# YichengDWu/tinyedm

Measured on AMD Instinct MI355X. Metric: train imgs/sec CIFAR-10 32x32 bf16, higher is better.
Workload: dtype bf16; 1 GPU; CIFAR-10 32x32 unconditional EDM2 U-Net (conf/cifar10.yaml, 35.6M params) full training step: diffuse+embed+denoiser fwd/bwd+loss+grad all-reduce+Adam+EMA; per_gpu_batch=128, global_batch=128, parallelism=dp1, conditional=False, step_launch=hipGraph replay, collective=none

## Files before the change

### tinyedm_amd/csrc/conv_wgrad3.hip

```cpp
#include "common.h"
#include <stdlib.h>

namespace {

typedef const __attribute__((address_space(1))) void* gptr_t;
typedef __attribute__((address_space(3))) void* lptr_t;
typedef __attribute__((address_space(3))) char lds_char;
typedef __attribute__((ext_vector_type(2))) unsigned u32x2_t;

constexpr int KP = 64;
constexpr int SUBB = KP * 64;
constexpr int TCO = 128, TCI = 64;
constexpr int TILE_FLOATS = 9 * TCO * TCI;
constexpr int MAXL = 48;
constexpr int DYRING = 3;

template <int LEADS>
struct Ring {
  static constexpr int XR = LEADS == 1 ? 4 : 8;
  static constexpr int MIRR = LEADS == 1 ? 2 : 4;
  static constexpr int XSLOTS = XR + MIRR;
  static constexpr size_t LDS = (size_t)DYRING * 4 * SUBB + (size_t)2 * XSLOTS * SUBB;
};

// ... 228 lines not shown
            kp = kpp; sw = wp; sh = hp; sn = np_;
            pix = pixel(valid);
            kq = kp;
            kp = kpn; sw = wn; sh = hn; sn = nn;
          }
          valid = valid && kq < ks1;
#pragma unroll
          for (int sub = 0; sub < 4; ++sub)
            if (valid && co0 + sub * 32 < Cout) dsrc[sub] = dY + pix * Cout + co0 + sub * 32 + dp * 8;
        }
      }
      char* const xdst = Xb + xslot * SUBB + wave * 1024;
      char* const ddst = dYb + ((t + 2) % DYRING) * (4 * SUBB) + wave * 1024;
      if constexpr (MF16) {
        const int slot = (t + LEADS) & (XR - 1);
        const int base_row = (slot < LEADS ? slot + XR : slot) * KP;
        const unsigned a_u = (unsigned)(uintptr_t)(lds_char*)dYb + (t % DYRING) * (4 * SUBB) + (cb * 2) * SUBB + krow16 * 64 + chan16;
        const unsigned b_u = (unsigned)(uintptr_t)(lds_char*)Xb + ib * (XSLOTS * SUBB) + (base_row + krow16) * 64 + chan16;
        unsigned tb[9];
#pragma unroll
        for (int tp = 0; tp < 9; ++tp) tb[tp] = b_u + ((tp / 3 - 1) * PW + (tp % 3 - 1)) * 64;
        u32x2_t A[2][4][2], Bf[6][2];
#define A_RD(set, c, ks2_)                                                                    \
  TR_RD(A[set][c][0], a_u, ((c) >> 1) * SUBB + ((c) & 1) * 32 + (ks2_) * 2048);               \
  TR_RD(A[set][c][1], a_u, ((c) >> 1) * SUBB + ((c) & 1) * 32 + (ks2_) * 2048 + 256);
        A_RD(0, 0, 0) A_RD(0, 1, 0) A_RD(0, 2, 0) A_RD(0, 3, 0)
        TR_RD(Bf[0][0], tb[0], 0); TR_RD(Bf[0][1], tb[0], 256);
        TR_RD(Bf[1][0], tb[0], 32); TR_RD(Bf[1][1], tb[0], 32 + 256);
        TR_RD(Bf[2][0], tb[1], 0); TR_RD(Bf[2][1], tb[1], 256);
        static_for<0, 36>([&](auto nc) {
          constexpr int n = decltype(nc)::value;
          constexpr int ks2 = n / 18, f = n % 18, tp = f / 2, b = f % 2;
          const unsigned au_ = a_u;
          constexpr int na = ((n - 3 <= 8 && 8 <= n - 1) ? 1 : 0) + ((n - 3 <= 10 && 10 <= n - 1) ? 1 : 0) +
                             ((n - 3 <= 12 && 12 <= n - 1) ? 1 : 0) + ((n - 3 <= 14 && 14 <= n - 1) ? 1 : 0);
          constexpr int cnt = n >= 33 ? (35 - n) * 2 : 4 + 2 * na;
          asm volatile("s_waitcnt lgkmcnt(%0)" ::"n"(cnt) : "memory");
          __builtin_amdgcn_sched_barrier(0);
          if constexpr (n == 1) { if (do_x) { dma16(xsrc0, xdst); if (xslot < MIRR) dma16(xsrc0, xdst + XR * SUBB); } __builtin_amdgcn_sched_barrier(0); }
          if constexpr (n == 5) { if (do_x) { dma16(xsrc1, xdst + XSLOTS * SUBB); if (xslot < MIRR) dma16(xsrc1, xdst + (XSLOTS + XR) * SUBB); } __builtin_amdgcn_sched_barrier(0); }
          if constexpr (n == 10) { if (do_dy) dma16(dsrc[0], ddst); __builtin_amdgcn_sched_barrier(0); }
          if constexpr (n == 14) { if (do_dy) dma16(dsrc[1], ddst + SUBB); __builtin_amdgcn_sched_barrier(0); }
          if constexpr (n == 19) { if (do_dy) dma16(dsrc[2], ddst + 2 * SUBB); __builtin_amdgcn_sched_barrier(0); }
          if constexpr (n == 23) { if (do_dy) dma16(dsrc[3], ddst + 3 * SUBB); __builtin_amdgcn_sched_barrier(0); }
          const bf16x8 bfr = frag_of(Bf[n % 6][0], Bf[n % 6][1]);
#pragma unroll
          for (int c = 0; c < 4; ++c) {
            const bf16x8 afr = frag_of(A[ks2 & 1][c][0], A[ks2 & 1][c][1]);
            if constexpr (tp < 8) asm volatile("v_mfma_f32_16x16x32_bf16 %0, %1, %2, %0" : "+a"(acc16[c][b][tp < 8 ? tp : 0]) : "v"(afr), "v"(bfr));
            else asm volatile("v_mfma_f32_16x16x32_bf16 %0, %1, %2, %0" : "+v"(accv16[c][b]) : "v"(afr), "v"(bfr));
            if constexpr (n + 3 < 36) {
              constexpr int m = n + 3, ksm = m / 18, fm = m % 18;
              if (c < 2) TR_RD(Bf[m % 6][c < 2 ? c : 0], tb[fm / 2], ksm * 2048 + (fm % 2) * 32 + (c < 2 ? c : 0) * 256);
            }
          }
          if constexpr (ks2 == 0 && b == 0 && tp >= 4 && tp <= 7) {
            constexpr int ca = tp - 4;
            TR_RD(A[1][ca][0], au_, (ca >> 1) * SUBB + (ca & 1) * 32 + 2048);
            TR_RD(A[1][ca][1], au_, (ca >> 1) * SUBB + (ca & 1) * 32 + 2048 + 256);
          }
        });
#undef A_RD
      } else if constexpr (!(ABL & 8)) {
        const int slot = (t + LEADS) & (XR - 1);
        const int base_row = (slot < LEADS ? slot + XR : slot) * KP;
        unsigned a_u = (unsigned)(uintptr_t)(lds_char*)dYb + (t % DYRING) * (4 * SUBB) + (cb * 2) * SUBB + krow_l * 64 + chan_b;
        const unsigned b_u = (unsigned)(uintptr_t)(lds_char*)Xb + ib * (XSLOTS * SUBB) + (base_row + krow_l) * 64 + chan_b;
        unsigned tb[9];
#pragma unroll
        for (int tp = 0; tp < 9; ++tp) tb[tp] = b_u + ((tp / 3 - 1) * PW + (tp % 3 - 1)) * 64;
        u32x2_t A[2][2][2], Bf[6][2];
        TR_RD(A[0][0][0], a_u, 0); TR_RD(A[0][0][1], a_u, 256);
        TR_RD(A[0][1][0], a_u, SUBB); TR_RD(A[0][1][1], a_u, SUBB + 256);
        TR_RD(Bf[0][0], tb[0], 0); TR_RD(Bf[0][1], tb[0], 256);
        TR_RD(Bf[1][0], tb[1], 0); TR_RD(Bf[1][1], tb[1], 256);
        TR_RD(Bf[2][0], tb[2], 0); TR_RD(Bf[2][1], tb[2], 256);
        static_for<0, 36>([&](auto nc) {
          constexpr int n = decltype(nc)::value;
          constexpr int ks = n / 9, p = n % 9;
          const unsigned au_ = a_u;
          constexpr int cnt = ks < 3 ? (p == 5 || p == 8 ? 6 : (p == 6 || p == 7 ? 8 : 4))
                                     : (p <= 6 ? 4 : (p == 7 ? 2 : 0));
          if constexpr (!(ABL & 32)) asm volatile("s_waitcnt lgkmcnt(%0)" ::"n"(cnt) : "memory");
          __builtin_amdgcn_sched_barrier(0);
          if constexpr (n == 1) { if (do_x) { dma16(xsrc0, xdst); if (xslot < MIRR) dma16(xsrc0, xdst + XR * SUBB); } __builtin_amdgcn_sched_barrier(0); }
          if constexpr (n == 5) { if (do_x) { dma16(xsrc1, xdst + XSLOTS * SUBB); if (xslot < MIRR) dma16(xsrc1, xdst + (XSLOTS + XR) * SUBB); } __builtin_amdgcn_sched_barrier(0); }
          if constexpr (n == 10) { if (do_dy) dma16(dsrc[0], ddst); __builtin_amdgcn_sched_barrier(0); }
          if constexpr (n == 14) { if (do_dy) dma16(dsrc[1], ddst + SUBB); __builtin_amdgcn_sched_barrier(0); }
          if constexpr (n == 19) { if (do_dy) dma16(dsrc[2], ddst + 2 * SUBB); __builtin_amdgcn_sched_barrier(0); }
          if constexpr (n == 23) { if (do_dy) dma16(dsrc[3], ddst + 3 * SUBB); __builtin_amdgcn_sched_barrier(0); }
          const bf16x8 bfr = frag_of(Bf[n % 6][0], Bf[n % 6][1]);
#pragma unroll
          for (int i = 0; i < 2; ++i) {
            const bf16x8 afr = frag_of(A[ks & 1][i][0], A[ks & 1][i][1]);
            if constexpr (!(ABL & 1)) {
              if constexpr (p < 8) asm volatile("v_mfma_f32_32x32x16_bf16 %0, %1, %2, %0" : "+a"(acc[i][p < 8 ? p : 0]) : "v"(afr), "v"(bfr));
              else asm volatile("v_mfma_f32_32x32x16_bf16 %0, %1, %2, %0" : "+v"(accv[i]) : "v"(afr), "v"(bfr));
            }
            if constexpr (n + 3 < 36) {
              constexpr int m = n + 3;
              TR_RD(Bf[m % 6][i], tb[m % 9], (m / 9) * 1024 + i * 256);
            }
          }
          if constexpr (ks < 3 && (p == 4 || p == 5)) {
            constexpr int ia = p - 4;
            TR_RD(A[(ks + 1) & 1][ia][0], au_, ia * SUBB + (ks + 1) * 1024);
            TR_RD(A[(ks + 1) & 1][ia][1], au_, ia * SUBB + (ks + 1) * 1024 + 256);
          }
        });
      } else {
        if (do_x) { dma16(xsrc0, xdst); if (xslot < MIRR) dma16(xsrc0, xdst + XR * SUBB); dma16(xsrc1, xdst + XSLOTS * SUBB); if (xslot < MIRR) dma16(xsrc1, xdst + (XSLOTS + XR) * SUBB); }
        if (do_dy) { dma16(dsrc[0], ddst); dma16(dsrc[1], ddst + SUBB); dma16(dsrc[2], ddst + 2 * SUBB); dma16(dsrc[3], ddst + 3 * SUBB); }
      }
    }
    asm volatile("s_nop 15\n\ts_nop 15" ::: "memory");
    if constexpr (MF16) {
#pragma unroll
      for (int c = 0; c < 4; ++c)
#pragma unroll
        for (int b = 0; b < 2; ++b)
#pragma unroll
          for (int tp = 0; tp < 9; ++tp) {
            float* base = out + ((long)tp * TCO + cb * 64 + c * 16 + 4 * lq) * TCI + ib * 32 + b * 16 + l15;
#pragma unroll
            for (int r = 0; r < 4; ++r) base[r * TCI] = (tp < 8) ? acc16[c][b][tp < 8 ? tp : 0][r] : accv16[c][b][r];
          }
    } else {
#pragma unroll
    for (int i = 0; i < 2; ++i)
#pragma unroll
      for (int tp = 0; tp < 9; ++tp) {
        float* base = out + ((long)tp * TCO + cb * 64 + i * 32) * TCI + ib * 32 + l31;
#pragma unroll
        for (int r = 0; r < 16; ++r)
          base[((r & 3) + 8 * (r >> 2) + 4 * lhi) * TCI] = (tp < 8) ? acc[i][tp < 8 ? tp : 0][r] : accv[i][r];
      }
    }
    pos += nst;
    if (pos >= g.L[li].stage0 + (long)g.L[li].ngroups * g.L[li].nst) ++li;
    __builtin_amdgcn_s_barrier();
  }
}

struct F3Layer {
  const float* w;
  float* grad;
  const int* perm;
  int O, I, Cin, tiles_ci, nst, row0;
  int gci, gco, nblk_ci, group0;
  int ksplit, tiles_co;
  float scale;
  int accumulate;
  long stage0;
};
struct F3Group {
  F3Layer L[MAXL];
  int nlayers, slots_per_member;
  long q;
  const float* work;
};

__device__ __forceinline__ float block_sum_f(float v, float* red) {
  v = wave_sum(v);
  const int lane = threadIdx.x & 63, wave = threadIdx.x >> 6;
  __syncthreads();
  if (lane == 0) red[wave] = v;
  __syncthreads();
  float s = 0.f;
  for (int i = 0; i < (int)(blockDim.x >> 6); ++i) s += red[i];
  return s;
}

__global__ __launch_bounds__(256) void k_wgrad3_finish(const F3Group* __restrict__ gp) {
  const F3Group& g = *gp;
  extern __shared__ __attribute__((aligned(16))) float gsm[];
  __shared__ float red[8];
  int li = 0;
  {
    int hi = g.nlayers - 1;
    while (li < hi) {
      const int mid = (li + hi + 1) >> 1;
      if ((int)blockIdx.x >= g.L[mid].row0) li = mid;
      else hi = mid - 1;
    }
  }
  const int r = blockIdx.x - g.L[li].row0;
  const int I = g.L[li].I, tiles_ci = g.L[li].tiles_ci, nst = g.L[li].nst;
  const int n = I * 9;
  const int mo = g.L[li].perm ? g.L[li].perm[r] : r;
  const float* __restrict__ row = g.L[li].w + (long)mo * n;
  const int tco = r / TCO, rl = r - tco * TCO;
  const float scale = g.L[li].scale;
  constexpr int WPF = 28;
  const bool pf = n <= WPF * 256;
  float wpre[WPF];
  if (pf) {
#pragma unroll
    for (int k = 0; k < WPF; ++k) {
      const int e = threadIdx.x + k * 256;
      wpre[k] = e < n ? row[e] : 0.f;
    }
  }
  const int items = tiles_ci * 9 * 16;
  for (int idx = threadIdx.x; idx < items; idx += blockDim.x) {
    const int c4 = idx & 15, tt = idx >> 4;
    const int tp = tt % 9, tci = tt / 9;
    const int gco = g.L[li].gco, gci = g.L[li].gci, ksplit = g.L[li].ksplit;
    f32x4 a = {0.f, 0.f, 0.f, 0.f};
    for (int ksh = 0; ksh < ksplit; ++ksh) {
      int grp, member;
      if (ksplit > 1) {
        const int v = ksh * (g.L[li].tiles_co * tiles_ci) + tco * tiles_ci + tci;
        grp = v >> 3;
        member = v & 7;
      } else {
        grp = (tco / gco) * g.L[li].nblk_ci + tci / gci;
        member = (tco % gco) * gci + tci % gci;
      }
      const long s0 = g.L[li].stage0 + (long)grp * nst;
      const int w_lo = (int)(s0 / g.q), w_hi = (int)((s0 + nst - 1) / g.q);
      const float* p = g.work + ((long)member * g.slots_per_member + w_lo + g.L[li].group0 + grp) * TILE_FLOATS +
                       ((long)tp * TCO + rl) * TCI + c4 * 4;
      for (int w = w_lo; w <= w_hi; ++w) {
        a += *reinterpret_cast<const f32x4*>(p);
        p += TILE_FLOATS;
      }
    }
    const int i0 = tci * TCI + c4 * 4;
#pragma unroll
    for (int j = 0; j < 4; ++j)
      if (i0 + j < I) gsm[(i0 + j) * 9 + tp] = a[j] * scale;
  }
  __syncthreads();
  float dot = 0.f, ss = 0.f;
  if (pf) {
#pragma unroll
    for (int k = 0; k < WPF; ++k) {
      const int e = threadIdx.x + k * 256;
      if (e < n) {
        dot += gsm[e] * wpre[k];
        ss += wpre[k] * wpre[k];
      }
    }
  } else {
    for (int e = threadIdx.x; e < n; e += blockDim.x) {
      const float wv = row[e];
      dot += gsm[e] * wv;
      ss += wv * wv;
    }
  }
  dot = block_sum_f(dot, red);
  ss = block_sum_f(ss, red);
  const float rn = sqrtf(ss);
  const float sqn = sqrtf((float)n);
  const float d = NORM_EPS + rn / sqn;
  const float c0 = 1.0f / (d * sqn);
  const float c1 = rn > 0.f ? dot / (d * rn * sqn) : 0.f;
  float* __restrict__ outp = g.L[li].grad + (long)mo * n;
  const int accumulate = g.L[li].accumulate;
  if (pf) {
#pragma unroll
    for (int k = 0; k < WPF; ++k) {
      const int e = threadIdx.x + k * 256;
      if (e < n) {
        const float v = c0 * (gsm[e] - wpre[k] * c1);
        outp[e] = accumulate ? outp[e] + v : v;
      }
    }
  } else {
    for (int e = threadIdx.x; e < n; e += blockDim.x) {
      const float v = c0 * (gsm[e] - row[e] * c1);
      outp[e] = accumulate ? outp[e] + v : v;
    }
  }
}

struct Plan {
  W3Group wg;
  F3Group fg;
  int leads, rows_total, ngroups_total, max_n;
  long work_floats;
};

}

extern "C" {
typedef struct {
  const void* X;
  const void* dY;
  const float* w;
  float* grad;
  const int* perm;
  int B, H, W, Cin, Cout, I;
  float scale;
  int accumulate;
} edm_wgrad3_item;
}


namespace {

int make_plan(const edm_wgrad3_item* it, int n, Plan& P) {
  EDM_REQUIRE(it && n > 0 && n <= MAXL, "wgrad3: need 1..%d layers per group, got %d", MAXL, n);
  P.leads = 0;
  long stage = 0;
  int group = 0, row = 0;
  P.max_n = 0;
  for (int k = 0; k < n; ++k) {
    const edm_wgrad3_item& a = it[k];
    EDM_REQUIRE(a.X && a.dY && a.w && a.grad, "wgrad3: null pointer in layer %d", k);
    EDM_REQUIRE(a.B > 0 && a.H > 0 && a.W > 0 && (long)a.B * (a.H + 1) * (a.W + 1) < (1L << 30), "wgrad3: bad B/H/W");
    EDM_REQUIRE(a.Cin > 0 && a.Cin % 32 == 0 && a.Cout > 0 && a.Cout % 32 == 0 && a.I > 0 && a.I <= a.Cin,
                "wgrad3: Cin=%d Cout=%d must be multiples of 32 (I=%d <= Cin)", a.Cin, a.Cout, a.I);
    EDM_REQUIRE(a.W + 2 <= 2 * KP, "wgrad3: W=%d > %d unsupported", a.W, 2 * KP - 2);
    EDM_REQUIRE((long)a.I * 9 * 4 <= 64 * 1024, "wgrad3: fan_in %d too large for the LDS row buffer", a.I * 9);
    const int leads = (a.W + 2 > KP) ? 2 : 1;
    EDM_REQUIRE(P.leads == 0 || P.leads == leads, "wgrad3: layers of one group must share the halo class (W <= 62 or W > 62)");
    P.leads = leads;
    W3Layer& L = P.wg.L[k];
    L.X = (const bf16*)a.X;
    L.dY = (const bf16*)a.dY;
    L.B = a.B; L.H = a.H; L.W = a.W; L.Cin = a.Cin; L.Cout = a.Cout;
    L.PW = a.W + 1;
    L.PH = a.H + 1;
    L.lead_rows = 2 + (leads * KP + L.PW - 1) / L.PW;
    L.kmult = (L.lead_rows + L.PH - 1) / L.PH;
    L.kbeg0 = (long)(L.lead_rows - 1) * L.PW + 1;
    L.kend = ((long)L.lead_rows + (long)a.B * L.PH) * L.PW;
    L.tiles_ci = (a.Cin + TCI - 1) / TCI;
    L.tiles_co = (a.Cout + TCO - 1) / TCO;
    L.gco = L.tiles_co >= 8 ? 8 : L.tiles_co >= 4 ? 4 : L.tiles_co >= 2 ? 2 : 1;
    {
      auto slots = [&](int gco) {
        const int gci = 8 / gco;
        return ((L.tiles_co + gco - 1) / gco) * ((L.tiles_ci + gci - 1) / gci);
      };
      static const bool search = [] { const char* e = getenv("EDM_W3_TEAMS"); return !(e && e[0] == '0'); }();
      int best = L.gco;
      for (int gco = 1; search && gco <= 8; gco *= 2)
        if (slots(gco) < slots(best)) best = gco;
      L.gco = best;
    }
    L.gci = 8 / L.gco;
    L.nblk_ci = (L.tiles_ci + L.gci - 1) / L.gci;
    L.ngroups = ((L.tiles_co + L.gco - 1) / L.gco) * L.nblk_ci;
    L.group0 = group;
    L.nst = (int)((L.kend - L.kbeg0 + KP - 1) / KP);
    L.ksplit = 1;
    {
      constexpr int W3_FLUSH_STAGES = 16;
      static const int smax = [] { const char* e = getenv("EDM_W3_KSPLIT"); return e ? atoi(e) : 8; }();
      const int T = L.tiles_co * L.tiles_ci;
      long best = (long)L.ngroups * (L.nst + W3_FLUSH_STAGES);
      for (int sp = 2; sp <= smax && sp <= 8; ++sp) {
        const int nst_s = (L.nst + sp - 1) / sp;
        if (nst_s < W3_FLUSH_STAGES) break;
        const long cost = (long)((T * sp + 7) / 8) * (nst_s + W3_FLUSH_STAGES);
        if (cost < best) { best = cost; L.ksplit = sp; }
      }
      if (L.ksplit > 1) {
        L.ngroups = (T * L.ksplit + 7) / 8;
        L.nst = (L.nst + L.ksplit - 1) / L.ksplit;
      }
    }
    L.stage0 = stage;
    F3Layer& F = P.fg.L[k];
    F.w = a.w; F.grad = a.grad; F.perm = a.perm;
    F.O = a.Cout; F.I = a.I; F.Cin = a.Cin; F.tiles_ci = L.tiles_ci; F.nst = L.nst; F.row0 = row;
    F.gci = L.gci; F.gco = L.gco; F.nblk_ci = L.nblk_ci; F.group0 = group;
    F.ksplit = L.ksplit; F.tiles_co = L.tiles_co;
    F.scale = a.scale; F.accumulate = a.accumulate; F.stage0 = stage;
    stage += (long)L.ngroups * L.nst;
    group += L.ngroups;
    row += a.Cout;
    if (a.I * 9 > P.max_n) P.max_n = a.I * 9;
  }
  constexpr int NXCD = 8, TPX_MAX = 4, QMIN = 8;
  int tpx = TPX_MAX;
  while (tpx > 1 && stage < (long)QMIN * NXCD * tpx) --tpx;
  const int teams = NXCD * tpx;
  const long q = (stage + teams - 1) / teams;
  P.wg.nlayers = P.fg.nlayers = n;
  P.wg.nwg = teams * 8;
  P.wg.tpx = tpx;
  P.wg.slots_per_member = P.fg.slots_per_member = teams + group;
  P.wg.total = stage;
  P.wg.q = P.fg.q = q;
  P.rows_total = row;
  P.ngroups_total = group;
  P.work_floats = (long)8 * (teams + group) * TILE_FLOATS;
  return EDM_OK;
}

}

extern "C" long edm_wgrad3_workspace(const edm_wgrad3_item* items, int n) {
  Plan P;
  if (make_plan(items, n, P) != EDM_OK) return -1;
  return P.work_floats * 4;
}

extern "C" int edm_wgrad3_plan_ksplit(const edm_wgrad3_item* items, int n, int* ksplit_out) {
  Plan P;
  const int rc = make_plan(items, n, P);
  if (rc != EDM_OK) return rc;
  EDM_REQUIRE(ksplit_out, "wgrad3_plan_ksplit: null output");
  for (int k = 0; k < n; ++k) ksplit_out[k] = P.wg.L[k].ksplit;
  return EDM_OK;
}

extern "C" long edm_wgrad3_table_bytes(void) { return (long)(sizeof(W3Group) + sizeof(F3Group)); }
extern "C" int edm_wgrad3_max_layers(void) { return MAXL; }

static thread_local hipEvent_t g_probe_start = nullptr, g_probe_end = nullptr;
extern "C" int edm_wgrad3_probe(void* ev_start, void* ev_end) {
  g_probe_start = (hipEvent_t)ev_start;
  g_probe_end = (hipEvent_t)ev_end;
  return EDM_OK;
}

extern "C" int edm_wgrad3_group(const edm_wgrad3_item* items, int n, void* workspace, long workspace_bytes,
                                void* table_host, void* table_dev, int defer_upload, hipStream_t st) {
  Plan P;
  const int rc = make_plan(items, n, P);
  if (rc != EDM_OK) return rc;
  EDM_REQUIRE(workspace && workspace_bytes >= P.work_floats * 4, "wgrad3: workspace too small (%ld < %ld bytes)",
              workspace_bytes, P.work_floats * 4);
  const bf16* zeros = (const bf16*)edm_zero_page();
  EDM_REQUIRE(zeros, "wgrad3: edm_init() has not been called on this device");
  P.wg.work = (float*)workspace;
  P.wg.zeros = zeros;
  P.fg.work = (const float*)workspace;
  static_assert(sizeof(W3Group) % 16 == 0, "F3Group must start aligned behind W3Group");
  {
    char stage[sizeof(W3Group) + sizeof(F3Group)];
    memcpy(stage, &P.wg, sizeof(W3Group));
    memcpy(stage + sizeof(W3Group), &P.fg, sizeof(F3Group));
    EDM_UPLOAD_TABLE(table_dev, table_host, stage, sizeof(stage), st, "wgrad3", defer_upload);
  }
  const W3Group* const wgp = (const W3Group*)table_dev;
  const F3Group* const fgp = (const F3Group*)((const char*)table_dev + sizeof(W3Group));
  static std::atomic<unsigned long long> set1{0}, set2{0};
  static const int abl = [] { const char* e = getenv("EDM_W3_ABLATE"); return e ? atoi(e) : 0; }();
  if (g_probe_start) (void)hipEventRecord(g_probe_start, st);
  if (P.leads == 1 && abl) {
    auto go = [&](auto kern) {
      (void)hipFuncSetAttribute(reinterpret_cast<const void*>(kern), hipFuncAttributeMaxDynamicSharedMemorySize, 160 * 1024);
      hipLaunchKernelGGL(kern, dim3(P.wg.nwg), dim3(256), Ring<1>::LDS, st, wgp);
    };
    switch (abl) {
      case 1: go(k_wgrad3<1, 1>); break;
      case 2: go(k_wgrad3<1, 2>); break;
      case 4: go(k_wgrad3<1, 4>); break;
      case 6: go(k_wgrad3<1, 6>); break;
      case 8: go(k_wgrad3<1, 8>); break;
      case 10: go(k_wgrad3<1, 10>); break;
      case 16: go(k_wgrad3<1, 16>); break;
      case 34: go(k_wgrad3<1, 34>); break;
      case 38: go(k_wgrad3<1, 38>); break;
      case 18: go(k_wgrad3<1, 18>); break;
      case 22: go(k_wgrad3<1, 22>); break;
      default: go(k_wgrad3<1, 14>); break;
    }
  } else {
    static const int mf16 = [] { const char* e = getenv("EDM_W3_MFMA16"); return e ? atoi(e) : 1; }();
    auto go = [&](auto kern, size_t lds, std::atomic<unsigned long long>& once) {
      edm_max_lds_once(reinterpret_cast<const void*>(kern), 160 * 1024, once);
      hipLaunchKernelGGL(kern, dim3(P.wg.nwg), dim3(256), lds, st, wgp);
    };
    static std::atomic<unsigned long long> set1m{0}, set2m{0};
    if (P.leads == 1) { if (mf16) go(k_wgrad3<1, 0, true>, Ring<1>::LDS, set1m); else go(k_wgrad3<1>, Ring<1>::LDS, set1); }
    else { if (mf16) go(k_wgrad3<2, 0, true>, Ring<2>::LDS, set2m); else go(k_wgrad3<2>, Ring<2>::LDS, set2); }
  }
  if (g_probe_end) (void)hipEventRecord(g_probe_end, st);
  g_probe_start = g_probe_end = nullptr;
  EDM_CHECK_LAUNCH("wgrad3");
  EDM_MAX_LDS(k_wgrad3_finish, 64 * 1024);
  hipLaunchKernelGGL(k_wgrad3_finish, dim3(P.rows_total), dim3(256), (size_t)P.max_n * 4, st, fgp);
  EDM_CHECK_LAUNCH("wgrad3_finish");
  return EDM_OK;
}
```

### tinyedm_amd/csrc/weights.hip

```cpp
#include "common.h"

namespace {

__device__ __forceinline__ float block_sum(float v, float* red) {
  v = wave_sum(v);
  const int lane = threadIdx.x & 63, wave = threadIdx.x >> 6;
  __syncthreads();
  if (lane == 0) red[wave] = v;
  __syncthreads();
  float s = 0.f;
  for (int i = 0; i < (int)(blockDim.x >> 6); ++i) s += red[i];
  return s;
}

__device__ __forceinline__ void prep_row(float* __restrict__ w, int O, int I, int taps, int Ipad,
                                         bf16* __restrict__ wp_fwd, bf16* __restrict__ wp_dgrad,
                                         float* __restrict__ w_hat, const int* __restrict__ perm,
                                         int normalize_inplace, int r, float* red) {
  const int mo = perm ? perm[r] : r;
  const int n = I * taps;
  float* row = w + (long)mo * n;
  const float rsn = rsqrtf((float)n);
  float ss = 0.f;
  for (int e = threadIdx.x; e < n; e += blockDim.x) ss += row[e] * row[e];
// ... 211 lines not shown
      const int o0 = r0 + og * 8;
      const int c = o0 >> 5, ks = (o0 >> 4) & 1, g = (o0 >> 3) & 1;
      const bf16* src = tile + (long)(og * 8) * n + (long)i * taps + t;
      bf16x8 v;
#pragma unroll
      for (int e = 0; e < 8; ++e) v[e] = src[(long)e * n];
      bf16* dst = d.dgrad + ((((long)((taps - 1 - t) * NC + c) * NCB + (i >> 5)) * 2 + ks) * 64 + g * 32 + (i & 31)) * 8;
      *reinterpret_cast<bf16x8*>(dst) = v;
    }
  }
  if (d.fwd && !frag_fwd) {
    for (int pair = wave; pair < rbc * taps; pair += 4) {
      const int rr = pair / taps, t = pair - rr * taps;
      bf16* dst = d.fwd + ((long)t * O + r0 + rr) * Ipad;
      const bf16* src = tile + (long)rr * n + t;
      if ((Ipad & 7) == 0) {
        for (int i8 = lane * 8; i8 < Ipad; i8 += 512) {
          bf16x8 v;
#pragma unroll
          for (int j = 0; j < 8; ++j) v[j] = (i8 + j < I) ? src[(i8 + j) * taps] : (bf16)0.f;
          *reinterpret_cast<bf16x8*>(dst + i8) = v;
        }
      } else {
        for (int i = lane; i < Ipad; i += 64) dst[i] = i < I ? src[i * taps] : (bf16)0.f;
      }
    }
  }
  if (d.dgrad && !frag_dgrad) {
    const bool vec = (rbc & 7) == 0 && (O & 7) == 0;
    for (int i = threadIdx.x; i < I; i += 256) {
      for (int t = 0; t < taps; ++t) {
        bf16* dst = d.dgrad + ((long)(taps - 1 - t) * I + i) * O + r0;
        const bf16* src = tile + i * taps + t;
        if (vec) {
          for (int c = 0; c < rbc; c += 8) {
            bf16x8 v;
#pragma unroll
            for (int j = 0; j < 8; ++j) v[j] = src[(long)(c + j) * n];
            *reinterpret_cast<bf16x8*>(dst + c) = v;
          }
        } else {
          for (int rr = 0; rr < rbc; ++rr) dst[rr] = src[(long)rr * n];
        }
      }
    }
  }
}

__global__ __launch_bounds__(1024) void k_wgrad_finish(const float* __restrict__ slabs, int S, const float* __restrict__ w,
                                                         float* __restrict__ grad, const int* __restrict__ perm, int O,
                                                         int I, int Ipad, int taps, float scale, int accumulate, int G) {
  extern __shared__ __attribute__((aligned(16))) float sm[];
  __shared__ float red[16];
  const int r = blockIdx.x;
  const int mo = perm ? perm[r] : r;
  const int n = I * taps;
  float* part = sm;
  float* g = sm + (long)G * n;
  const float* row = w + (long)mo * n;
  const long slab_stride = (long)taps * O * Ipad;
  if ((I & 3) == 0 && (Ipad & 3) == 0) {
    const int I4 = I >> 2, E4 = taps * I4;
    if (S <= 3) {
      const int items = E4;
      for (int idx0 = threadIdx.x; idx0 < items * G; idx0 += 4 * blockDim.x) {
        f32x4 acc4[4];
        int e4s[4], sgs[4];
#pragma unroll
        for (int u = 0; u < 4; ++u) {
          const int idx = idx0 + u * blockDim.x;
          const bool ok = idx < items * G;
          const int sg = ok ? idx / E4 : 0, e4 = ok ? idx - sg * E4 : 0;
          e4s[u] = ok ? e4 : -1;
          sgs[u] = sg;
          const int t = e4 / I4, i = (e4 - t * I4) * 4;
          const float* sp = slabs + ((long)t * O + r) * Ipad + i;
          f32x4 a = {0.f, 0.f, 0.f, 0.f};
          if (ok)
            for (int sl = sg; sl < S; sl += G) a += *reinterpret_cast<const f32x4*>(sp + (long)sl * slab_stride);
          acc4[u] = a;
        }
#pragma unroll
        for (int u = 0; u < 4; ++u)
          if (e4s[u] >= 0) *reinterpret_cast<f32x4*>(part + (long)sgs[u] * n + e4s[u] * 4) = acc4[u];
      }
    } else
    for (int idx = threadIdx.x; idx < E4 * G; idx += blockDim.x) {
      const int sg = idx / E4, e4 = idx - sg * E4;
      const int t = e4 / I4, i = (e4 - t * I4) * 4;
      const float* sp = slabs + ((long)t * O + r) * Ipad + i;
      f32x4 a = {0.f, 0.f, 0.f, 0.f};
      int s = sg;
      for (; s + 7 * G < S; s += 8 * G) {
        f32x4 v[8];
#pragma unroll
        for (int u = 0; u < 8; ++u) v[u] = *reinterpret_cast<const f32x4*>(sp + (long)(s + u * G) * slab_stride);
#pragma unroll
        for (int u = 0; u < 8; ++u) a += v[u];
      }
      for (; s < S; s += G) a += *reinterpret_cast<const f32x4*>(sp + (long)s * slab_stride);
      *reinterpret_cast<f32x4*>(part + (long)sg * n + e4 * 4) = a;
    }
  } else {
    for (int idx = threadIdx.x; idx < n * G; idx += blockDim.x) {
      const int sg = idx / n, e = idx - sg * n;
      const int t = e / I, i = e - t * I;
      const float* sp = slabs + ((long)t * O + r) * Ipad + i;
      float a = 0.f;
      for (int s = sg; s < S; s += G) a += sp[(long)s * slab_stride];
      part[(long)sg * n + e] = a;
    }
  }
  __syncthreads();
  float dot = 0.f, ss = 0.f;
  for (int e = threadIdx.x; e < n; e += blockDim.x) {
    float a = 0.f;
    for (int sg = 0; sg < G; ++sg) a += part[(long)sg * n + e];
    a *= scale;
    const int t = e / I, i = e - t * I;
    const float wv = row[i * taps + t];
    g[i * taps + t] = a;
    dot += a * wv;
    ss += wv * wv;
  }
  dot = block_sum(dot, red);
  ss = block_sum(ss, red);
  const float rn = sqrtf(ss);
  const float sqn = sqrtf((float)n);
  const float d = NORM_EPS + rn / sqn;
  const float c0 = 1.0f / (d * sqn);
  const float c1 = rn > 0.f ? dot / (d * rn * sqn) : 0.f;
  __syncthreads();
  float* out = grad + (long)mo * n;
  for (int e = threadIdx.x; e < n; e += blockDim.x) {
    float v = c0 * (g[e] - row[e] * c1);
    out[e] = accumulate ? out[e] + v : v;
  }
}

constexpr int MAXF = 40;
struct FinItem {
  const float* slabs;
  const float* w;
  float* grad;
  const int* perm;
  int S, O, I, Ipad, taps, G, row0;
  float scale;
  int accumulate, pad;
};
struct FinGroup {
  FinItem it[MAXF];
  int n, prefetch;
};
__global__ __launch_bounds__(512) void k_wgrad_finish_multi(const FinGroup* __restrict__ gp) {
  const FinGroup& g = *gp;
  extern __shared__ __attribute__((aligned(16))) float smm[];
  __shared__ float red[16];
  int k = 0;
  while (k + 1 < g.n && (int)blockIdx.x >= g.it[k + 1].row0) ++k;
  const int r = blockIdx.x - g.it[k].row0;
  const float* __restrict__ slabs = g.it[k].slabs;
  const int S = g.it[k].S, O = g.it[k].O, I = g.it[k].I, Ipad = g.it[k].Ipad, taps = g.it[k].taps, G = g.it[k].G;
  const float scale = g.it[k].scale;
  const int mo = g.it[k].perm ? g.it[k].perm[r] : r;
  const int n = I * taps;
  float* part = smm;
  float* gm = smm + (long)G * n;
  const float* row = g.it[k].w + (long)mo * n;
  const long slab_stride = (long)taps * O * Ipad;
  constexpr int WPF = 2;
  const bool pf = g.prefetch && n <= WPF * 512;
  float* out = g.it[k].grad + (long)mo * n;
  const int accumulate = g.it[k].accumulate;
  float wpre[WPF] = {0.f, 0.f}, opre[WPF] = {0.f, 0.f};
  if (pf) {
#pragma unroll
    for (int q = 0; q < WPF; ++q) {
      const int e = threadIdx.x + q * 512;
      if (e < n) {
        wpre[q] = row[e];
        if (accumulate) opre[q] = out[e];
      }
    }
  }
  if ((I & 3) == 0 && (Ipad & 3) == 0) {
    const int I4 = I >> 2, E4 = taps * I4;
    for (int idx = threadIdx.x; idx < E4 * G; idx += blockDim.x) {
      const int sg = idx / E4, e4 = idx - sg * E4;
      const int t = e4 / I4, i = (e4 - t * I4) * 4;
      const float* sp = slabs + ((long)t * O + r) * Ipad + i;
      f32x4 a = {0.f, 0.f, 0.f, 0.f};
      int s = sg;
      for (; s + 3 * G < S; s += 4 * G) {
        f32x4 v[4];
#pragma unroll
        for (int u = 0; u < 4; ++u) v[u] = *reinterpret_cast<const f32x4*>(sp + (long)(s + u * G) * slab_stride);
#pragma unroll
        for (int u = 0; u < 4; ++u) a += v[u];
      }
      for (; s < S; s += G) a += *reinterpret_cast<const f32x4*>(sp + (long)s * slab_stride);
      *reinterpret_cast<f32x4*>(part + (long)sg * n + e4 * 4) = a;
    }
  } else {
    for (int idx = threadIdx.x; idx < n * G; idx += blockDim.x) {
      const int sg = idx / n, e = idx - sg * n;
      const int t = e / I, i = e - t * I;
      const float* sp = slabs + ((long)t * O + r) * Ipad + i;
      float a = 0.f;
      for (int s = sg; s < S; s += G) a += sp[(long)s * slab_stride];
      part[(long)sg * n + e] = a;
    }
  }
  __syncthreads();
  float dot = 0.f, ss = 0.f;
  if (pf && taps == 1) {
#pragma unroll
    for (int q = 0; q < WPF; ++q) {
      const int e = threadIdx.x + q * 512;
      if (e < n) {
        float a = 0.f;
        for (int sg = 0; sg < G; ++sg) a += part[(long)sg * n + e];
        a *= scale;
        gm[e] = a;
        dot += a * wpre[q];
        ss += wpre[q] * wpre[q];
      }
    }
  } else {
    for (int e = threadIdx.x; e < n; e += blockDim.x) {
      float a = 0.f;
      for (int sg = 0; sg < G; ++sg) a += part[(long)sg * n + e];
      a *= scale;
      const int t = e / I, i = e - t * I;
      const float wv = row[i * taps + t];
      gm[i * taps + t] = a;
      dot += a * wv;
      ss += wv * wv;
    }
  }
  dot = block_sum(dot, red);
  ss = block_sum(ss, red);
  const float rn = sqrtf(ss);
  const float sqn = sqrtf((float)n);
  const float d = NORM_EPS + rn / sqn;
  const float c0 = 1.0f / (d * sqn);
  const float c1 = rn > 0.f ? dot / (d * rn * sqn) : 0.f;
  __syncthreads();
  if (pf) {
#pragma unroll
    for (int q = 0; q < WPF; ++q) {
      const int e = threadIdx.x + q * 512;
      if (e < n) {
        const float v = c0 * (gm[e] - wpre[q] * c1);
        out[e] = accumulate ? opre[q] + v : v;
      }
    }
  } else {
    for (int e = threadIdx.x; e < n; e += blockDim.x) {
      const float v = c0 * (gm[e] - row[e] * c1);
      out[e] = accumulate ? out[e] + v : v;
    }
  }
}

}

extern "C" {
typedef struct {
  const float* slabs;
  const float* w;
  float* grad;
  const int* perm;
  int S, O, I, Ipad, taps;
  float scale;
  int accumulate;
} edm_finish_item;
}

extern "C" long edm_wgrad_finish_multi_table_bytes(void) { return (long)sizeof(FinGroup); }

extern "C" int edm_wgrad_finish_multi(const edm_finish_item* items, int n, void* table_host, void* table_dev, int defer_upload, hipStream_t st) {
  EDM_REQUIRE(items && n > 0 && n <= MAXF, "wgrad_finish_multi: need 1..%d tensors, got %d", MAXF, n);
  FinGroup g;
  g.n = n;
  static const int prefetch = [] { const char* e = getenv("EDM_FIN_PREFETCH"); return e ? atoi(e) : 1; }();
  g.prefetch = prefetch;
  int row = 0;
  size_t lds = 0;
  for (int k = 0; k < n; ++k) {
    const edm_finish_item& a = items[k];
    EDM_REQUIRE(a.slabs && a.w && a.grad && a.S > 0 && a.O > 0 && a.I > 0 && a.taps > 0 && a.Ipad >= a.I,
                "wgrad_finish_multi: bad item %d", k);
    const int nn = a.I * a.taps;
    const int E = ((a.I & 3) == 0 && (a.Ipad & 3) == 0) ? nn / 4 : nn;
    int G = 1;
    while (G < 8 && 2 * G <= a.S && E * 2 * G <= 512 && (long)(2 * G + 1) * nn * 4 <= 96 * 1024) G *= 2;
    EDM_REQUIRE((long)(G + 1) * nn * 4 <= 128 * 1024, "wgrad_finish_multi: fan_in %d too large for the LDS row buffer", nn);
    g.it[k] = FinItem{a.slabs, a.w, a.grad, a.perm, a.S, a.O, a.I, a.Ipad, a.taps, G, row, a.scale, a.accumulate, 0};
    row += a.O;
    const size_t need = (size_t)(G + 1) * nn * sizeof(float);
    if (need > lds) lds = need;
  }
  EDM_MAX_LDS(k_wgrad_finish_multi, 128 * 1024);
  EDM_UPLOAD_TABLE(table_dev, table_host, &g, sizeof(FinGroup), st, "wgrad_finish_multi", defer_upload);
  hipLaunchKernelGGL(k_wgrad_finish_multi, dim3(row), dim3(512), lds, st, (const FinGroup*)table_dev);
  EDM_CHECK_LAUNCH("wgrad_finish_multi");
  return EDM_OK;
}

extern "C" int edm_weight_prep(float* w, int O, int I, int taps, int Ipad, void* wp_fwd, void* wp_dgrad,
                               float* w_hat, const int* perm, int normalize_inplace, hipStream_t st) {
  EDM_REQUIRE(w && O > 0 && I > 0 && taps > 0 && Ipad >= I, "weight_prep: bad args O=%d I=%d taps=%d Ipad=%d", O, I, taps, Ipad);
  hipLaunchKernelGGL(k_weight_prep, dim3(O), dim3(256), 0, st, w, O, I, taps, Ipad, (bf16*)wp_fwd, (bf16*)wp_dgrad,
                     w_hat, perm, normalize_inplace);
  EDM_CHECK_LAUNCH("weight_prep");
  return EDM_OK;
}

extern "C" int edm_weight_prep_multi(const void* descs, const int* groups, int n_groups, int lds_bytes,
                                     int normalize_inplace, hipStream_t st) {
  EDM_REQUIRE(descs && groups && n_groups > 0 && lds_bytes > 0 && lds_bytes <= 128 * 1024, "weight_prep_multi: bad args");
  static_assert(sizeof(PrepDesc) == 64, "PrepDesc layout");
  EDM_MAX_LDS(k_weight_prep_multi, 128 * 1024);
  hipLaunchKernelGGL(k_weight_prep_multi, dim3(n_groups), dim3(256), (size_t)lds_bytes, st, (const PrepDesc*)descs,
                     (const int2*)groups, normalize_inplace);
  EDM_CHECK_LAUNCH("weight_prep_multi");
  return EDM_OK;
}

extern "C" int edm_wgrad_finish(const float* slabs, int S, const float* w, float* grad, const int* perm, int O, int I,
                                int Ipad, int taps, float scale, int accumulate, hipStream_t st) {
  EDM_REQUIRE(slabs && w && grad && S > 0 && O > 0 && I > 0 && taps > 0 && Ipad >= I, "wgrad_finish: bad args");
  const int n = I * taps;
  EDM_REQUIRE((long)n * 4 <= 64 * 1024, "wgrad_finish: fan_in %d too large for the LDS row buffer", n);
  const int E = ((I & 3) == 0 && (Ipad & 3) == 0) ? n / 4 : n;
  int G = 1;
  while (G < 8 && 2 * G <= S && E * 2 * G <= 1024 && (long)(2 * G + 1) * n * 4 <= 96 * 1024) G *= 2;
  const int items = E * G;
  const int passes = (items + 1023) / 1024;
  int threads = ((items + passes - 1) / passes + 63) / 64 * 64;
  if (threads < 64) threads = 64;
  if (threads > 1024) threads = 1024;
  const size_t lds = (size_t)(G + 1) * n * sizeof(float);
  EDM_MAX_LDS(k_wgrad_finish, 128 * 1024);
  hipLaunchKernelGGL(k_wgrad_finish, dim3(O), dim3(threads), lds, st, slabs, S, w, grad, perm, O, I, Ipad, taps, scale,
                     accumulate, G);
  EDM_CHECK_LAUNCH("wgrad_finish");
  return EDM_OK;
}
```

Measured before the change: 9995 img/s.

## Add streaming weight-gradient finish kernels with wave-per-row reduction for 1x1 layers

Adds a new 3x3 wgrad finish kernel that runs 576 threads per row, caps the per-group partial-tile loop with a host-computed maxt, and unrolls the vectorised loads 8 deep. It also adds a 1x1 finish path that gives each wave one output row, reducing the slabs in registers with wave_sum instead of LDS and block barriers, packing 8 rows per block. Both paths are on by default and can be disabled with an environment variable. The aim is to cut memory latency and sync overhead in the gradient finish stage. The cost is higher register pressure and more code paths to maintain.

```diff
diff --git a/tinyedm_amd/csrc/conv_wgrad3.hip b/tinyedm_amd/csrc/conv_wgrad3.hip
--- a/tinyedm_amd/csrc/conv_wgrad3.hip
+++ b/tinyedm_amd/csrc/conv_wgrad3.hip
@@ -404,6 +404,7 @@
   float scale;
   int accumulate;
   long stage0;
+  int maxt;
 };
 struct F3Group {
   F3Layer L[MAXL];
@@ -517,6 +518,120 @@
       if (e < n) {
         const float v = c0 * (gsm[e] - wpre[k] * c1);
         outp[e] = accumulate ? outp[e] + v : v;
+      }
+    }
+  } else {
+    for (int e = threadIdx.x; e < n; e += blockDim.x) {
+      const float v = c0 * (gsm[e] - row[e] * c1);
+      outp[e] = accumulate ? outp[e] + v : v;
+    }
+  }
+}
+
+constexpr int F3_THREADS = 576, F3_UJ = 8;
+
+__global__ __launch_bounds__(F3_THREADS) void k_wgrad3_finish_stream(const F3Group* __restrict__ gp) {
+  const F3Group& g = *gp;
+  extern __shared__ __attribute__((aligned(16))) float gsm[];
+  __shared__ float red[16];
+  int li = 0;
+  {
+    int hi = g.nlayers - 1;
+    while (li < hi) {
+      const int mid = (li + hi + 1) >> 1;
+      if ((int)blockIdx.x >= g.L[mid].row0) li = mid;
+      else hi = mid - 1;
+    }
+  }
+  const int r = blockIdx.x - g.L[li].row0;
+  const int I = g.L[li].I, tiles_ci = g.L[li].tiles_ci, nst = g.L[li].nst;
+  const int n = I * 9;
+  const int mo = g.L[li].perm ? g.L[li].perm[r] : r;
+  const float* __restrict__ row = g.L[li].w + (long)mo * n;
+  float* __restrict__ outp = g.L[li].grad + (long)mo * n;
+  const int accumulate = g.L[li].accumulate;
+  const int tco = r / TCO, rl = r - tco * TCO;
+  const float scale = g.L[li].scale;
+  constexpr int WPF = 13;
+  const bool pf = n <= WPF * F3_THREADS;
+  float wpre[WPF], opre[WPF];
+  if (pf) {
+#pragma unroll
+    for (int k = 0; k < WPF; ++k) {
+      const int e = threadIdx.x + k * F3_THREADS;
+      wpre[k] = e < n ? row[e] : 0.f;
+      opre[k] = (accumulate && e < n) ? outp[e] : 0.f;
+    }
+  }
+  const int items = tiles_ci * 9 * 16;
+  const int gco = g.L[li].gco, gci = g.L[li].gci, ksplit = g.L[li].ksplit, maxt = g.L[li].maxt;
+  const f32x4 zero4 = {0.f, 0.f, 0.f, 0.f};
+  for (int idx = threadIdx.x; idx < items; idx += F3_THREADS) {
+    const int c4 = idx & 15, tt = idx >> 4;
+    const int tp = tt % 9, tci = tt / 9;
+    f32x4 a = zero4;
+    for (int ksh = 0; ksh < ksplit; ++ksh) {
+      int grp, member;
+      if (ksplit > 1) {
+        const int v = ksh * (g.L[li].tiles_co * tiles_ci) + tco * tiles_ci + tci;
+        grp = v >> 3;
+        member = v & 7;
+      } else {
+        grp = (tco / gco) * g.L[li].nblk_ci + tci / gci;
+        member = (tco % gco) * gci + tci % gci;
+      }
+      const long s0 = g.L[li].stage0 + (long)grp * nst;
+      const int w_lo = (int)(s0 / g.q), w_hi = (int)((s0 + nst - 1) / g.q);
+      const int cnt = w_hi - w_lo + 1;
+      const float* p = g.work + ((long)member * g.slots_per_member + w_lo + g.L[li].group0 + grp) * TILE_FLOATS +
+                       ((long)tp * TCO + rl) * TCI + c4 * 4;
+      for (int j0 = 0; j0 < maxt; j0 += F3_UJ) {
+        f32x4 v[F3_UJ];
+#pragma unroll
+        for (int u = 0; u < F3_UJ; ++u)
+          v[u] = j0 + u < cnt ? *reinterpret_cast<const f32x4*>(p + (long)(j0 + u) * TILE_FLOATS) : zero4;
+#pragma unroll
+        for (int u = 0; u < F3_UJ; ++u)
+          if (j0 + u < cnt) a += v[u];
+      }
+    }
+    const int i0 = tci * TCI + c4 * 4;
+#pragma unroll
+    for (int j = 0; j < 4; ++j)
+      if (i0 + j < I) gsm[(i0 + j) * 9 + tp] = a[j] * scale;
+  }
+  __syncthreads();
+  float dot = 0.f, ss = 0.f;
+  if (pf) {
+#pragma unroll
+    for (int k = 0; k < WPF; ++k) {
+      const int e = threadIdx.x + k * F3_THREADS;
+      if (e < n) {
+        dot += gsm[e] * wpre[k];
+        ss += wpre[k] * wpre[k];
+      }
+    }
+  } else {
+    for (int e = threadIdx.x; e < n; e += blockDim.x) {
+      const float wv = row[e];
+      dot += gsm[e] * wv;
+      ss += wv * wv;
+    }
+  }
+  dot = block_sum_f(dot, red);
+  ss = block_sum_f(ss, red);
+  const float rn = sqrtf(ss);
+  const float sqn = sqrtf((float)n);
+  const float d = NORM_EPS + rn / sqn;
+  const float c0 = 1.0f / (d * sqn);
+  const float c1 = rn > 0.f ? dot / (d * rn * sqn) : 0.f;
+  if (pf) {
+#pragma unroll
+    for (int k = 0; k < WPF; ++k) {
+      const int e = threadIdx.x + k * F3_THREADS;
+      if (e < n) {
+        const float v = c0 * (gsm[e] - wpre[k] * c1);
+        outp[e] = accumulate ? opre[k] + v : v;
       }
     }
   } else {
@@ -638,6 +753,16 @@
   P.wg.slots_per_member = P.fg.slots_per_member = teams + group;
   P.wg.total = stage;
   P.wg.q = P.fg.q = q;
+  for (int k = 0; k < n; ++k) {
+    const W3Layer& L = P.wg.L[k];
+    int maxt = 1;
+    for (int grp = 0; grp < L.ngroups; ++grp) {
+      const long s0 = L.stage0 + (long)grp * L.nst;
+      const int t = (int)((s0 + L.nst - 1) / q - s0 / q) + 1;
+      if (t > maxt) maxt = t;
+    }
+    P.fg.L[k].maxt = maxt;
+  }
   P.rows_total = row;
   P.ngroups_total = group;
   P.work_floats = (long)8 * (teams + group) * TILE_FLOATS;
@@ -727,8 +852,18 @@
   if (g_probe_end) (void)hipEventRecord(g_probe_end, st);
   g_probe_start = g_probe_end = nullptr;
   EDM_CHECK_LAUNCH("wgrad3");
-  EDM_MAX_LDS(k_wgrad3_finish, 64 * 1024);
-  hipLaunchKernelGGL(k_wgrad3_finish, dim3(P.rows_total), dim3(256), (size_t)P.max_n * 4, st, fgp);
+  bool stream;
+  {
+    const char* e = getenv("EDM_FIN_STREAM");
+    stream = !(e && e[0] == '0');
+  }
+  if (stream) {
+    EDM_MAX_LDS(k_wgrad3_finish_stream, 64 * 1024);
+    hipLaunchKernelGGL(k_wgrad3_finish_stream, dim3(P.rows_total), dim3(F3_THREADS), (size_t)P.max_n * 4, st, fgp);
+  } else {
+    EDM_MAX_LDS(k_wgrad3_finish, 64 * 1024);
+    hipLaunchKernelGGL(k_wgrad3_finish, dim3(P.rows_total), dim3(256), (size_t)P.max_n * 4, st, fgp);
+  }
   EDM_CHECK_LAUNCH("wgrad3_finish");
   return EDM_OK;
 }
diff --git a/tinyedm_amd/csrc/weights.hip b/tinyedm_amd/csrc/weights.hip
--- a/tinyedm_amd/csrc/weights.hip
+++ b/tinyedm_amd/csrc/weights.hip
@@ -387,26 +387,27 @@
   FinItem it[MAXF];
   int n, prefetch;
 };
-__global__ __launch_bounds__(512) void k_wgrad_finish_multi(const FinGroup* __restrict__ gp) {
-  const FinGroup& g = *gp;
-  extern __shared__ __attribute__((aligned(16))) float smm[];
-  __shared__ float red[16];
-  int k = 0;
-  while (k + 1 < g.n && (int)blockIdx.x >= g.it[k + 1].row0) ++k;
-  const int r = blockIdx.x - g.it[k].row0;
-  const float* __restrict__ slabs = g.it[k].slabs;
-  const int S = g.it[k].S, O = g.it[k].O, I = g.it[k].I, Ipad = g.it[k].Ipad, taps = g.it[k].taps, G = g.it[k].G;
-  const float scale = g.it[k].scale;
-  const int mo = g.it[k].perm ? g.it[k].perm[r] : r;
+template <bool EXACT>
+__device__ __forceinline__ float fin_add(float old, float v) {
+  if constexpr (EXACT) asm("" : "+v"(v));
+  return old + v;
+}
+
+template <bool EXACT>
+__device__ __forceinline__ void finish_row_block(const FinItem& it, int prefetch, int r, float* smm, float* red) {
+  const float* __restrict__ slabs = it.slabs;
+  const int S = it.S, O = it.O, I = it.I, Ipad = it.Ipad, taps = it.taps, G = it.G;
+  const float scale = it.scale;
+  const int mo = it.perm ? it.perm[r] : r;
   const int n = I * taps;
   float* part = smm;
   float* gm = smm + (long)G * n;
-  const float* row = g.it[k].w + (long)mo * n;
+  const float* row = it.w + (long)mo * n;
   const long slab_stride = (long)taps * O * Ipad;
   constexpr int WPF = 2;
-  const bool pf = g.prefetch && n <= WPF * 512;
-  float* out = g.it[k].grad + (long)mo * n;
-  const int accumulate = g.it[k].accumulate;
+  const bool pf = prefetch && n <= WPF * 512;
+  float* out = it.grad + (long)mo * n;
+  const int accumulate = it.accumulate;
   float wpre[WPF] = {0.f, 0.f}, opre[WPF] = {0.f, 0.f};
   if (pf) {
 #pragma unroll
@@ -487,14 +488,146 @@
       const int e = threadIdx.x + q * 512;
       if (e < n) {
         const float v = c0 * (gm[e] - wpre[q] * c1);
-        out[e] = accumulate ? opre[q] + v : v;
+        out[e] = accumulate ? fin_add<EXACT>(opre[q], v) : v;
       }
     }
   } else {
     for (int e = threadIdx.x; e < n; e += blockDim.x) {
       const float v = c0 * (gm[e] - row[e] * c1);
-      out[e] = accumulate ? out[e] + v : v;
-    }
+      out[e] = accumulate ? fin_add<EXACT>(out[e], v) : v;
+    }
+  }
+}
+
+__global__ __launch_bounds__(512) void k_wgrad_finish_multi(const FinGroup* __restrict__ gp) {
+  const FinGroup& g = *gp;
+  extern __shared__ __attribute__((aligned(16))) float smm[];
+  __shared__ float red[16];
+  int k = 0;
+  while (k + 1 < g.n && (int)blockIdx.x >= g.it[k + 1].row0) ++k;
+  finish_row_block<false>(g.it[k], g.prefetch, blockIdx.x - g.it[k].row0, smm, red);
+}
+
+constexpr int FIN_RPB = 8;
+constexpr int FIN_U = 8;
+constexpr int FIN_MAXI = 1024;
+
+__device__ __forceinline__ f32x4 ld4(const float* p) { return *reinterpret_cast<const f32x4*>(p); }
+template <int N>
+struct FinC { static constexpr int value = N; };
+
+template <int NC>
+__device__ __forceinline__ void finish_row_wave(const FinItem& it, int r) {
+  const int lane = threadIdx.x & 63;
+  const int S = it.S, I = it.I, Ipad = it.Ipad;
+  const float scale = it.scale;
+  const int accumulate = it.accumulate;
+  const int mo = it.perm ? it.perm[r] : r;
+  const float* __restrict__ row = it.w + (long)mo * I;
+  float* __restrict__ out = it.grad + (long)mo * I;
+  const float* __restrict__ sp = it.slabs + (long)r * Ipad;
+  const long slab_stride = (long)it.O * Ipad;
+  const int C = I >> 2;
+  const f32x4 zero4 = {0.f, 0.f, 0.f, 0.f};
+  f32x4 wv[NC], ov[NC], a[NC];
+#pragma unroll
+  for (int j = 0; j < NC; ++j) {
+    const int c = lane + 64 * j;
+    wv[j] = c < C ? ld4(row + 4 * c) : zero4;
+    ov[j] = (accumulate && c < C) ? ld4(out + 4 * c) : zero4;
+    a[j] = zero4;
+  }
+  auto sum_cols = [&](auto kc, auto uc, int j0) {
+    constexpr int K = decltype(kc)::value, U = decltype(uc)::value;
+    const float* p[K];
+    bool ok[K];
+#pragma unroll
+    for (int q = 0; q < K; ++q) {
+      const int c = lane + 64 * (j0 + q);
+      ok[q] = c < C;
+      p[q] = sp + 4 * c;
+    }
+    for (int s = 0; s < S; s += U) {
+      f32x4 v[K][U];
+      if (s + U <= S) {
+#pragma unroll
+        for (int u = 0; u < U; ++u)
+#pragma unroll
+          for (int q = 0; q < K; ++q) v[q][u] = ok[q] ? ld4(p[q] + (long)(s + u) * slab_stride) : zero4;
+#pragma unroll
+        for (int u = 0; u < U; ++u)
+#pragma unroll
+          for (int q = 0; q < K; ++q) a[j0 + q] += v[q][u];
+      } else {
+#pragma unroll
+        for (int u = 0; u < U; ++u)
+#pragma unroll
+          for (int q = 0; q < K; ++q) v[q][u] = (ok[q] && s + u < S) ? ld4(p[q] + (long)(s + u) * slab_stride) : zero4;
+#pragma unroll
+        for (int u = 0; u < U; ++u)
+          if (s + u < S) {
+#pragma unroll
+            for (int q = 0; q < K; ++q) a[j0 + q] += v[q][u];
+          }
+      }
+    }
+  };
+  if constexpr (NC == 2) {
+    if (C <= 64) sum_cols(FinC<1>{}, FinC<2 * FIN_U>{}, 0);
+    else sum_cols(FinC<2>{}, FinC<FIN_U>{}, 0);
+  } else {
+#pragma unroll
+    for (int j = 0; j < NC; ++j)
+      if (64 * j < C) sum_cols(FinC<1>{}, FinC<FIN_U>{}, j);
+  }
+  float dot = 0.f, ss = 0.f;
+#pragma unroll
+  for (int j = 0; j < NC; ++j) {
+    a[j] *= scale;
+#pragma unroll
+    for (int e = 0; e < 4; ++e) {
+      dot += a[j][e] * wv[j][e];
+      ss += wv[j][e] * wv[j][e];
+    }
+  }
+  dot = wave_sum(dot);
+  ss = wave_sum(ss);
+  const int n = I;
+  const float rn = sqrtf(ss);
+  const float sqn = sqrtf((float)n);
+  const float d = NORM_EPS + rn / sqn;
+  const float c0 = 1.0f / (d * sqn);
+  const float c1 = rn > 0.f ? dot / (d * rn * sqn) : 0.f;
+#pragma unroll
+  for (int j = 0; j < NC; ++j) {
+    const int c = lane + 64 * j;
+    if (c < C) {
+      f32x4 o;
+#pragma unroll
+      for (int e = 0; e < 4; ++e) {
+        const float v = c0 * (a[j][e] - wv[j][e] * c1);
+        o[e] = accumulate ? fin_add<true>(ov[j][e], v) : v;
+      }
+      *reinterpret_cast<f32x4*>(out + 4 * c) = o;
+    }
+  }
+}
+
+__global__ __launch_bounds__(512, 4) void k_wgrad_finish_multi_stream(const FinGroup* __restrict__ gp) {
+  const FinGroup& g = *gp;
+  extern __shared__ __attribute__((aligned(16))) float smm[];
+  __shared__ float red[16];
+  int k = 0;
+  while (k + 1 < g.n && (int)blockIdx.x >= g.it[k + 1].row0) ++k;
+  const int b = blockIdx.x - g.it[k].row0;
+  if (g.it[k].pad) {
+    const int r = b * FIN_RPB + __builtin_amdgcn_readfirstlane((int)(threadIdx.x >> 6));
+    if (r < g.it[k].O) {
+      if (g.it[k].I <= 512) finish_row_wave<2>(g.it[k], r);
+      else finish_row_wave<4>(g.it[k], r);
+    }
+  } else {
+    finish_row_block<true>(g.it[k], g.prefetch, b, smm, red);
   }
 }
 
@@ -520,6 +653,11 @@
   g.n = n;
   static const int prefetch = [] { const char* e = getenv("EDM_FIN_PREFETCH"); return e ? atoi(e) : 1; }();
   g.prefetch = prefetch;
+  bool stream;
+  {
+    const char* e = getenv("EDM_FIN_STREAM");
+    stream = !(e && e[0] == '0');
+  }
   int row = 0;
   size_t lds = 0;
   for (int k = 0; k < n; ++k) {
@@ -531,14 +669,25 @@
     int G = 1;
     while (G < 8 && 2 * G <= a.S && E * 2 * G <= 512 && (long)(2 * G + 1) * nn * 4 <= 96 * 1024) G *= 2;
     EDM_REQUIRE((long)(G + 1) * nn * 4 <= 128 * 1024, "wgrad_finish_multi: fan_in %d too large for the LDS row buffer", nn);
-    g.it[k] = FinItem{a.slabs, a.w, a.grad, a.perm, a.S, a.O, a.I, a.Ipad, a.taps, G, row, a.scale, a.accumulate, 0};
+    const bool wave_row = stream && a.taps == 1 && (a.I & 3) == 0 && (a.Ipad & 3) == 0 && a.I <= FIN_MAXI &&
+                          (((uintptr_t)a.slabs | (uintptr_t)a.w | (uintptr_t)a.grad) & 15) == 0;
+    g.it[k] = FinItem{a.slabs, a.w, a.grad, a.perm, a.S, a.O, a.I, a.Ipad, a.taps, G, row, a.scale, a.accumulate, wave_row};
+    if (wave_row) {
+      row += (a.O + FIN_RPB - 1) / FIN_RPB;
+      continue;
+    }
     row += a.O;
     const size_t need = (size_t)(G + 1) * nn * sizeof(float);
     if (need > lds) lds = need;
   }
-  EDM_MAX_LDS(k_wgrad_finish_multi, 128 * 1024);
   EDM_UPLOAD_TABLE(table_dev, table_host, &g, sizeof(FinGroup), st, "wgrad_finish_multi", defer_upload);
-  hipLaunchKernelGGL(k_wgrad_finish_multi, dim3(row), dim3(512), lds, st, (const FinGroup*)table_dev);
+  if (stream) {
+    EDM_MAX_LDS(k_wgrad_finish_multi_stream, 128 * 1024);
+    hipLaunchKernelGGL(k_wgrad_finish_multi_stream, dim3(row), dim3(512), lds, st, (const FinGroup*)table_dev);
+  } else {
+    EDM_MAX_LDS(k_wgrad_finish_multi, 128 * 1024);
+    hipLaunchKernelGGL(k_wgrad_finish_multi, dim3(row), dim3(512), lds, st, (const FinGroup*)table_dev);
+  }
   EDM_CHECK_LAUNCH("wgrad_finish_multi");
   return EDM_OK;
 }
```

New measurement: 9939 img/s. No clear change (-0.6%).
